# dyollb/segmantic

Measured on AMD Instinct MI355X. Metric: 3D UNet train voxels/s on 128^3 bf16, higher is better.
Workload: dtype bf16

## Files before the change

### segmantic_amd/csrc/conv.hip

```cpp
#include "conv_fwd_impl.h"
#include "conv_ring_impl.h"
#include "conv_ks_impl.h"
#include "convt_ps_impl.h"
#include "conv_bnbwd_impl.h"

namespace segmi {

int conv_s2_bnbwd_bf16(const ConvBnBwdParams& p, hipStream_t st);
int conv_s2_bnbwd_f16(const ConvBnBwdParams& p, hipStream_t st);

int conv_mfma_f32(const ConvParams& p, int ksize, int stride, hipStream_t st);
int conv_mfma_bf16(const ConvParams& p, int ksize, int stride, hipStream_t st);
int conv_mfma_f16(const ConvParams& p, int ksize, int stride, hipStream_t st);
int convt_mfma_f32(const ConvTParams& p, hipStream_t st);
int convt_mfma_bf16(const ConvTParams& p, hipStream_t st);
int convt_mfma_f16(const ConvTParams& p, hipStream_t st);
static inline int conv_mfma_dt(int dtype, const ConvParams& p, int ksize, int stride, hipStream_t st) {
  if (dtype == SEGMI_F32) return conv_mfma_f32(p, ksize, stride, st);
  return dtype == SEGMI_F16 ? conv_mfma_f16(p, ksize, stride, st) : conv_mfma_bf16(p, ksize, stride, st);
}
static inline int convt_mfma_dt(int dtype, const ConvTParams& p, hipStream_t st) {
  if (dtype == SEGMI_F32) return convt_mfma_f32(p, st);
  return dtype == SEGMI_F16 ? convt_mfma_f16(p, st) : convt_mfma_bf16(p, st);
}
int bn_stats_launch(int dtype, const segmi_act* x, float* partials, hipStream_t st, const BiasFin* bias_fin = nullptr);
int bn_stats_rows_for(const segmi_act* x);
int stats_reserve_rows();
static inline int bn_finalize_with(const float* partials, int rows, int c, const segmi_bn_fin* f, hipStream_t st) {
  return segmi_bn_finalize(partials, rows, c, f->count, f->gamma, f->beta, f->running_mean, f->running_var,
                           f->momentum, f->eps, f->mean, f->invstd, f->scale, f->shift, st);
}
bool conv_small_ok(int cin, int cout, int ksize);
int conv_small_fwd(int dtype, const segmi_act* in, const segmi_act* out, const float* w,
                   const float* bias, const float* alpha, const segmi_act* res, float* stats,
                   int stride, hipStream_t st, const segmi_act* out2 = nullptr,
                   const float* w2 = nullptr, const float* bias2 = nullptr,
                   const segmi_bn_fin* fin = nullptr, const segmi_windows* win = nullptr);
int conv_small_fwd_rows(const segmi_act* out);

struct DirectParams {
  const void* in;
  void* out;
  const float* w;
  const float* bias;
  const float* alpha;
  const void* res;
  int N, Di, Hi, Wi, Do, Ho, Wo, Cin, Cout, ldi, ldo, ldr;
  int ks, stride, kind;
};

template <typename T>
__global__ void conv_direct_kernel(DirectParams p) {
  const int64_t total = (int64_t)p.N * p.Do * p.Ho * p.Wo * p.Cout;
  const int pad = (p.ks - 1) / 2, nt = p.ks * p.ks * p.ks;
  const T* in = (const T*)p.in;
  for (int64_t e = blockIdx.x * (int64_t)blockDim.x + threadIdx.x; e < total;
       e += (int64_t)gridDim.x * blockDim.x) {
    const int co = e % p.Cout;
    int64_t v = e / p.Cout;
    const int ox = v % p.Wo; v /= p.Wo;
    const int oy = v % p.Ho; v /= p.Ho;
    const int oz = v % p.Do;
    const int n = v / p.Do;
    float acc = 0.f;
    for (int kd = 0; kd < p.ks; ++kd) {
      const int z = oz * p.stride - pad + kd;
      if ((unsigned)z >= (unsigned)p.Di) continue;
      for (int kh = 0; kh < p.ks; ++kh) {
        const int y = oy * p.stride - pad + kh;
        if ((unsigned)y >= (unsigned)p.Hi) continue;
        for (int kw = 0; kw < p.ks; ++kw) {
          const int x = ox * p.stride - pad + kw;
          if ((unsigned)x >= (unsigned)p.Wi) continue;
          const int tap = (kd * p.ks + kh) * p.ks + kw;
          const T* ip = in + ((((int64_t)n * p.Di + z) * p.Hi + y) * p.Wi + x) * p.ldi;
          if (p.kind == 0) {
            const float* wp = p.w + ((int64_t)co * p.Cin) * nt + tap;
            for (int ci = 0; ci < p.Cin; ++ci) acc = fmaf(Elem<T>::ld(ip + ci), wp[(int64_t)ci * nt], acc);
          } else {
            const float* wp = p.w + (int64_t)co * nt + (nt - 1 - tap);
            for (int ci = 0; ci < p.Cin; ++ci)
              acc = fmaf(Elem<T>::ld(ip + ci), wp[(int64_t)ci * p.Cout * nt], acc);
          }
        }
      }
    }
    if (p.bias) acc += p.bias[co];
    if (p.alpha) acc = acc > 0.f ? acc : (*p.alpha) * acc;
    const int64_t vox = (((int64_t)n * p.Do + oz) * p.Ho + oy) * p.Wo + ox;
    if (p.res) acc += Elem<T>::ld((const T*)p.res + vox * p.ldr + co);
    Elem<T>::st((T*)p.out + vox * p.ldo + co, acc);
  }
}

template <typename T>
__global__ void convt_direct_kernel(DirectParams p) {
  const int64_t total = (int64_t)p.N * p.Do * p.Ho * p.Wo * p.Cout;
  const T* in = (const T*)p.in;
  for (int64_t e = blockIdx.x * (int64_t)blockDim.x + threadIdx.x; e < total;
       e += (int64_t)gridDim.x * blockDim.x) {
    const int co = e % p.Cout;
    int64_t v = e / p.Cout;
    const int ox = v % p.Wo; v /= p.Wo;
    const int oy = v % p.Ho; v /= p.Ho;
    const int oz = v % p.Do;
    const int n = v / p.Do;
    float acc = 0.f;
    for (int kd = 0; kd < 3; ++kd) {
      const int tz = oz + 1 - kd;
      if (tz < 0 || (tz & 1) || (tz >> 1) >= p.Di) continue;
      for (int kh = 0; kh < 3; ++kh) {
        const int ty = oy + 1 - kh;
        if (ty < 0 || (ty & 1) || (ty >> 1) >= p.Hi) continue;
        for (int kw = 0; kw < 3; ++kw) {
          const int tx = ox + 1 - kw;
          if (tx < 0 || (tx & 1) || (tx >> 1) >= p.Wi) continue;
          const int tap = (kd * 3 + kh) * 3 + kw;
          const T* ip = in + ((((int64_t)n * p.Di + (tz >> 1)) * p.Hi + (ty >> 1)) * p.Wi + (tx >> 1)) * p.ldi;
          const float* wp = p.w + (int64_t)co * 27 + tap;
          for (int ci = 0; ci < p.Cin; ++ci)
            acc = fmaf(Elem<T>::ld(ip + ci), wp[(int64_t)ci * p.Cout * 27], acc);
        }
      }
    }
    if (p.bias) acc += p.bias[co];
    if (p.alpha) acc = acc > 0.f ? acc : (*p.alpha) * acc;
    const int64_t vox = (((int64_t)n * p.Do + oz) * p.Ho + oy) * p.Wo + ox;
    if (p.res) acc += Elem<T>::ld((const T*)p.res + vox * p.ldr + co);
    Elem<T>::st((T*)p.out + vox * p.ldo + co, acc);
  }
}

static inline bool mfma_ok(int cin, int cout) { return cin % 16 == 0 && cout % 16 == 0; }

static inline int out_extent(int in, int ks, int stride) {
  const int pad = (ks - 1) / 2;
  return (in + 2 * pad - ks) / stride + 1;
}

}

using namespace segmi;

static inline bool small_fwd_eligible(int dtype, const segmi_act* in, const segmi_act* out, int ksize) {
  const int es = dtype_size(dtype);
  return conv_small_ok(in->c, out->c, ksize) && out->ld % 4 == 0 &&
         ((uintptr_t)out->data % (4 * es)) == 0;
}

extern "C" {

int segmi_conv3d_stats_rows(int dtype, const segmi_act* in, const segmi_act* out, int ksize,
                            int stride) {
  if (!in || !out) return 0;
  if (mfma_ok(in->c, out->c)) {
    if (conv_ring_ok(dtype, in->c, ksize, stride, out))
      return conv_ring_rows(dtype, in->c, out) + stats_reserve_rows();
    if (conv_ks_ok(dtype, in->c, ksize, stride)) return conv_ks_rows(out) + stats_reserve_rows();
    return conv_mfma_rows(out, stride) + stats_reserve_rows();
  }
  if (small_fwd_eligible(dtype, in, out, ksize)) return conv_small_fwd_rows(out) + stats_reserve_rows();
  return bn_stats_rows_for(out) + stats_reserve_rows();
}

int segmi_conv3d_pair_ok(int dtype, const segmi_act* in, const segmi_act* out_a,
                         const segmi_act* out_b) {
  if (!act_ok(in) || !act_ok(out_a) || !act_ok(out_b)) return 0;
  if (!dtype_ok(dtype)) return 0;
  return !mfma_ok(in->c, out_a->c) && small_fwd_eligible(dtype, in, out_a, 3) &&
         small_fwd_eligible(dtype, in, out_b, 3) && out_a->c == out_b->c && out_a->n == out_b->n &&
         out_a->d == out_b->d && out_a->h == out_b->h && out_a->w == out_b->w;
}

int segmi_conv3d_fwd_pair(int dtype, const segmi_act* in, const segmi_act* out_a, const float* w_a,
                          const float* bias_a, const float* prelu_alpha_a, float* stats_partials_a,
                          const segmi_act* out_b, const float* w_b, const float* bias_b, int stride,
                          const segmi_bn_fin* stats_fin_a, const segmi_windows* windows, void* stream) {
  SEGMI_CHECK_ARG(!stats_fin_a || (stats_partials_a && bn_fin_ok(stats_fin_a)),
                  "conv3d_fwd_pair: stats_fin_a needs stats_partials_a and its output pointers");
  if (windows) {
    const int es = dtype_size(dtype);
    bool ok = in && in->c == 1 && in->ld == 1 && windows->count == in->n && windows->count >= 1 && windows->count <= 32 &&
              windows->row_stride >= in->w && windows->row_stride % 4 == 0 && in->w % 4 == 0 &&
              windows->plane_stride >= (int64_t)windows->row_stride * in->h && windows->plane_stride % 4 == 0 &&
              ((uintptr_t)in->data % (4 * es)) == 0;
    for (int i = 0; ok && i < windows->count; ++i) ok = windows->offset[i] >= 0 && windows->offset[i] % 4 == 0;
    SEGMI_CHECK_ARG(ok, "conv3d_fwd_pair: bad window views (single channel, <= 32 windows, 4-element aligned "
                        "offsets and strides)");
  }
  SEGMI_CHECK_ARG(segmi_conv3d_pair_ok(dtype, in, out_a, out_b),
                  "conv3d_fwd_pair: not a small-Cin k3 pair (ask segmi_conv3d_pair_ok first)");
  SEGMI_CHECK_ARG(w_a && w_b && (stride == 1 || stride == 2), "conv3d_fwd_pair: bad arguments");
  SEGMI_CHECK_ARG(in->n == out_a->n && out_a->d == out_extent(in->d, 3, stride) &&
                      out_a->h == out_extent(in->h, 3, stride) && out_a->w == out_extent(in->w, 3, stride),
                  "conv3d_fwd_pair: output extent does not match the input");
  SEGMI_CHECK_ARG(!(stats_partials_a && prelu_alpha_a),
                  "conv3d_fwd_pair: fused statistics are taken before PReLU");
  return conv_small_fwd(dtype, in, out_a, w_a, bias_a, prelu_alpha_a, nullptr, stats_partials_a,
                        stride, (hipStream_t)stream, out_b, w_b, bias_b, stats_fin_a, windows);
}

int segmi_conv3d_split_act_ok(int dtype, const segmi_act* in, const segmi_act* out, int ksize,
                              int stride) {
  if (!act_ok(in) || !act_ok(out) || !dtype_ok(dtype)) return 0;
  return mfma_ok(in->c, out->c) && ksize == 3 && stride == 2 && !conv_ks_ok(dtype, in->c, ksize, stride) &&
         !conv_ring_ok(dtype, in->c, ksize, stride, out);
}

int segmi_conv3d_fwd_split_act(int dtype, const segmi_act* in, const segmi_act* out, const void* packed,
                               const float* bias, const float* prelu_alpha, int act_channels, int ksize,
                               int stride, const float* bias_b, float* stats_partials,
                               const segmi_bn_fin* stats_fin, void* stream) {
  SEGMI_CHECK_ARG(segmi_conv3d_split_act_ok(dtype, in, out, ksize, stride),
                  "conv3d_fwd_split_act: layer not eligible (ask segmi_conv3d_split_act_ok)");
  SEGMI_CHECK_ARG(packed && act_channels > 0 && act_channels % 16 == 0 && act_channels <= out->c,
                  "conv3d_fwd_split_act: act_channels must be a multiple of 16 within the output channels");
  SEGMI_CHECK_ARG(in->n == out->n && out->d == out_extent(in->d, ksize, stride) &&
                      out->h == out_extent(in->h, ksize, stride) && out->w == out_extent(in->w, ksize, stride),
                  "conv3d_fwd_split_act: output extent does not match the input");
  const int es = dtype_size(dtype);
  SEGMI_CHECK_ARG(in->ld % (16 / es) == 0 && out->ld % 4 == 0 && ((uintptr_t)in->data % 16) == 0 &&
                      ((uintptr_t)out->data % (4 * es)) == 0,
                  "conv3d_fwd_split_act: MFMA path needs 16-byte aligned input rows");
  ConvParams p{};
  p.in = in->data; p.out = out->data; p.wfrag = packed; p.bias = bias; p.alpha = prelu_alpha;
  p.N = in->n; p.Di = in->d; p.Hi = in->h; p.Wi = in->w;
  p.Do = out->d; p.Ho = out->h; p.Wo = out->w;
  p.Cin = in->c; p.Cout = out->c; p.ldi = in->ld; p.ldo = out->ld;
  p.nchunks = in->c / pick_ck(dtype, in->c);
  p.ntiles_total = out->c / 16;
  p.act_tiles = act_channels / 16;
  p.bias2 = bias_b;
  if (stats_partials) {
    p.stats = stats_partials;
    p.stats_tiles = act_channels / 16;
    if (stats_fin) { p.fin_on = 1; p.bfin = bn_fin_from(stats_fin, act_channels); }
  } else {
    SEGMI_CHECK_ARG(!stats_fin, "conv3d_fwd_split_act: stats_fin needs stats_partials");
  }
  hipStream_t st = (hipStream_t)stream;
  return conv_mfma_dt(dtype, p, ksize, stride, st);
}

const char* segmi_conv3d_fwd_kernel_name(int dtype, const segmi_act* in, const segmi_act* out,
                                         int ksize, int stride) {
  static thread_local char buf[96];
  if (!act_ok(in) || !act_ok(out)) return "invalid";
  const char* dt = dtype == SEGMI_BF16 ? "bf16" : dtype == SEGMI_F16 ? "f16" : "f32";
  if (mfma_ok(in->c, out->c)) {
    const int ck = pick_ck(dtype, in->c);
    if (conv_ring_ok(dtype, in->c, ksize, stride, out)) {
      if (conv_ring3_shape_ok(in->c, out->c, in->data, out->data, in->d, in->h, in->w, in->ld, out->d, out->h, out->w, out->ld,
                              out->ld, out->ld))
        snprintf(buf, sizeof buf, "conv_ring3_kernel<%s, CK=16> (LDS-DMA ring)", dt);
      else
        snprintf(buf, sizeof buf, "conv_ring2_kernel<%s, CK=%d, NT=%d>", dt, ck,
                 ck == 32 && (out->c / 16) % 2 == 0 ? 2 : 1);
    }
    else if (conv_ks_ok(dtype, in->c, ksize, stride))
      snprintf(buf, sizeof buf, "conv_fwd_ks_kernel<%s, k%d s%d>", dt, ksize, stride);
    else
      snprintf(buf, sizeof buf, "conv_fwd_mfma_kernel<%s, CK=%d, k%d s%d>", dt, ck, ksize, stride);
    return buf;
  }
  if (small_fwd_eligible(dtype, in, out, ksize)) snprintf(buf, sizeof buf, "conv_small_fwd_kernel<%s>", dt);
  else snprintf(buf, sizeof buf, "conv_direct_kernel<%s>", dt);
  return buf;
}

int segmi_conv3d_in_affine_ok(int dtype, const segmi_act* in, const segmi_act* out, int ksize,
                              int stride) {
  if (!act_ok(in) || !act_ok(out) || !dtype_h16(dtype) || !mfma_ok(in->c, out->c)) return 0;
  return ksize == 3 && stride == 1 && conv_ring_ok(dtype, in->c, ksize, stride, out) ? 1 : 0;
}

int segmi_conv3d_bn_bwd_sums_ok(int dtype, const segmi_act* in, const segmi_act* out, int ksize,
                                int stride) {
  if (!act_ok(in) || !act_ok(out) || !dtype_h16(dtype)) return 0;
  return ((in->c == 16 && out->c == 16) || (in->c == 32 && out->c == 32)) && ksize == 3 && stride == 1 &&
                 conv_ring_ok(dtype, in->c, ksize, stride, out) ? 1 : 0;
}

int segmi_bn_act_bwd_apply_conv_ok(int dtype, const segmi_act* dy, const segmi_act* x, const segmi_act* dx,
                                   const segmi_act* out) {
  if (!dtype_h16(dtype) || !act_ok(dy) || !act_ok(x) || !act_ok(dx) || !act_ok(out)) return 0;
  const segmi_act* a3[3] = {dy, x, dx};
  for (const segmi_act* a : a3) {
    if (a->n != dy->n || a->d != dy->d || a->h != dy->h || a->w != dy->w || a->c != 16) return 0;
    if (a->ld % 8 != 0 || ((uintptr_t)a->data % 16) != 0) return 0;
  }
  if (out->n != dy->n || out->d != out_extent(dy->d, 3, 2) || out->h != out_extent(dy->h, 3, 2) ||
      out->w != out_extent(dy->w, 3, 2))
    return 0;
  if (!(out->c == 16 || out->c == 32 || out->c == 64) || out->ld % 4 != 0 || ((uintptr_t)out->data % 8) != 0)
    return 0;
  const int64_t vox = (int64_t)dy->d * dy->h * dy->w;
  if (vox * dy->ld * 2 >= (1ll << 31) || vox * x->ld * 2 >= (1ll << 31) || vox * dx->ld * 2 >= (1ll << 31)) return 0;
  return out->w >= 16 ? 1 : 0;
}

int segmi_bn_act_bwd_apply_conv(int dtype, const segmi_act* dy, const segmi_act* x, const segmi_act* dx,
                                const float* mean, const float* invstd, const float* gamma, const float* beta,
                                const float* prelu_alpha, const float* coef, const segmi_act* out,
                                const void* packed, void* stream) {
  SEGMI_CHECK_ARG(segmi_bn_act_bwd_apply_conv_ok(dtype, dy, x, dx, out) && mean && invstd && coef && packed,
                  "bn_act_bwd_apply_conv: not eligible (ask segmi_bn_act_bwd_apply_conv_ok) or bad arguments");
  SEGMI_CHECK_ARG(dx->data != dy->data && dx->data != x->data,
                  "bn_act_bwd_apply_conv: dx must not alias dy or x (halo voxels are re-read by neighbouring tiles)");
  ConvBnBwdParams p{};
  p.dy = dy->data; p.x = x->data; p.dx = dx->data; p.out = out->data; p.wfrag = packed;
  p.mean = mean; p.invstd = invstd; p.gamma = gamma; p.beta = beta; p.alpha = prelu_alpha; p.coef = coef;
  p.N = dy->n; p.Di = dy->d; p.Hi = dy->h; p.Wi = dy->w; p.Do = out->d; p.Ho = out->h; p.Wo = out->w;
  p.Cout = out->c; p.ldy = dy->ld; p.ldx = x->ld; p.lddx = dx->ld; p.ldo = out->ld;
  p.ntiles_total = out->c / 16;
  return dtype == SEGMI_F16 ? conv_s2_bnbwd_f16(p, (hipStream_t)stream) : conv_s2_bnbwd_bf16(p, (hipStream_t)stream);
}

int segmi_conv3d_fwd(int dtype, const segmi_act* in, const segmi_act* out, const void* packed,
                     const float* w_src, int w_kind, const float* bias,
                     const float* prelu_alpha, const segmi_act* residual,
                     float* stats_partials, int ksize, int stride, const segmi_in_affine* in_tf,
                     const segmi_bn_bwd_sums* bn_bwd, const segmi_bn_fin* stats_fin, void* stream) {
  SEGMI_CHECK_ARG(!stats_fin || (stats_partials && bn_fin_ok(stats_fin)),
                  "conv3d: stats_fin needs stats_partials and its output pointers");
  if (bn_bwd && bn_bwd->fin)
    SEGMI_CHECK_ARG(bn_bwd->fin->count > 0 && bn_bwd->fin->coef, "conv3d: bn_bwd->fin needs count and coef");
  if (bn_bwd)
    SEGMI_CHECK_ARG(bn_bwd->x && act_ok(bn_bwd->x) && bn_bwd->mean && bn_bwd->invstd && bn_bwd->partials &&
                        segmi_conv3d_bn_bwd_sums_ok(dtype, in, out, ksize, stride) && !prelu_alpha &&
                        !stats_partials && bn_bwd->x->n == out->n && bn_bwd->x->d == out->d &&
                        bn_bwd->x->h == out->h && bn_bwd->x->w == out->w && bn_bwd->x->c == out->c &&
                        bn_bwd->x->ld % 4 == 0 && ((uintptr_t)bn_bwd->x->data % 8) == 0,
                    "conv3d: this launch cannot take BatchNorm-backward sums (ask segmi_conv3d_bn_bwd_sums_ok)");
  if (in_tf)
    SEGMI_CHECK_ARG(in_tf->scale && in_tf->shift && segmi_conv3d_in_affine_ok(dtype, in, out, ksize, stride),
                    "conv3d: this layer cannot take an input transform (ask segmi_conv3d_in_affine_ok)");
  SEGMI_CHECK_ARG(dtype_ok(dtype), "conv3d: bad dtype %d", dtype);
  SEGMI_CHECK_ARG(act_ok(in) && act_ok(out), "conv3d: bad activation view");
  SEGMI_CHECK_ARG((ksize == 1 || ksize == 3) && (stride == 1 || stride == 2),
                  "conv3d: unsupported ksize/stride %d/%d", ksize, stride);
  SEGMI_CHECK_ARG(!(ksize == 1 && stride != 1), "conv3d: k1 is stride 1 only");
  SEGMI_CHECK_ARG(in->n == out->n && out->d == out_extent(in->d, ksize, stride) &&
                      out->h == out_extent(in->h, ksize, stride) &&
                      out->w == out_extent(in->w, ksize, stride),
                  "conv3d: output extent [%d,%d,%d,%d] does not match input [%d,%d,%d,%d] k%d s%d",
                  out->n, out->d, out->h, out->w, in->n, in->d, in->h, in->w, ksize, stride);
  if (residual)
    SEGMI_CHECK_ARG(act_ok(residual) && residual->n == out->n && residual->d == out->d &&
                        residual->h == out->h && residual->w == out->w && residual->c == out->c,
                    "conv3d: residual shape mismatch");
  hipStream_t st = (hipStream_t)stream;
  const int es = dtype_size(dtype);
  if (mfma_ok(in->c, out->c)) {
    SEGMI_CHECK_ARG(packed, "conv3d: MFMA path needs a fragment-packed weight (segmi_wpack)");
    SEGMI_CHECK_ARG(in->ld % (16 / es) == 0 && out->ld % 4 == 0 &&
                        ((uintptr_t)in->data % 16) == 0 && ((uintptr_t)out->data % (4 * es)) == 0,
                    "conv3d: MFMA path needs 16-byte aligned input rows");
    if (residual)
      SEGMI_CHECK_ARG(residual->ld % 4 == 0 && ((uintptr_t)residual->data % (4 * es)) == 0,
                      "conv3d: residual rows must be 4-element aligned");
    ConvParams p{};
    p.in = in->data; p.out = out->data; p.wfrag = packed; p.bias = bias; p.alpha = prelu_alpha;
    p.res = residual ? residual->data : nullptr; p.stats = stats_partials;
    p.N = in->n; p.Di = in->d; p.Hi = in->h; p.Wi = in->w;
    p.Do = out->d; p.Ho = out->h; p.Wo = out->w;
    p.Cin = in->c; p.Cout = out->c; p.ldi = in->ld; p.ldo = out->ld;
    p.ldr = residual ? residual->ld : 0;
    p.nchunks = in->c / pick_ck(dtype, in->c);
    p.ntiles_total = out->c / 16;
    if (in_tf) { p.in_scale = in_tf->scale; p.in_shift = in_tf->shift; p.in_alpha = in_tf->prelu_alpha; }
    if (bn_bwd) {
      p.bx = bn_bwd->x->data; p.ldbx = bn_bwd->x->ld; p.bmean = bn_bwd->mean; p.binvstd = bn_bwd->invstd;
      p.bgamma = bn_bwd->gamma; p.bbeta = bn_bwd->beta; p.balpha = bn_bwd->prelu_alpha;
      p.bpart = bn_bwd->partials;
      SEGMI_CHECK_ARG((int64_t)p.Ho * p.Wo * p.ldbx < (1ll << 31), "conv3d: plane too large for 32-bit offsets");
      if (bn_bwd->fin) {
        p.fin_on = 1;
        p.bbfin = BnBwdFin{out->c, bn_bwd->fin->count, bn_bwd->fin->dgamma, bn_bwd->fin->dbeta,
                           bn_bwd->fin->dalpha, bn_bwd->fin->coef};
      }
    }
    if (stats_fin) { p.fin_on = 1; p.bfin = bn_fin_from(stats_fin, out->c); }
    return conv_mfma_dt(dtype, p, ksize, stride, st);
  }
  SEGMI_CHECK_ARG(w_src, "conv3d: direct path (channels not multiples of 16) needs w_src");
  SEGMI_CHECK_ARG(w_kind == 0 || w_kind == 1, "conv3d: bad w_kind %d", w_kind);
  SEGMI_CHECK_ARG(!(stats_partials && small_fwd_eligible(dtype, in, out, ksize) && w_kind != 0),
                  "conv3d: fused statistics on a small-Cin layer need the forward weight kind");
  if (small_fwd_eligible(dtype, in, out, ksize) && w_kind == 0 &&
      (!residual || (residual->ld % 4 == 0 && ((uintptr_t)residual->data % (4 * es)) == 0))) {
    SEGMI_CHECK_ARG(!stats_partials || (!prelu_alpha && !residual),
                    "conv3d: fused statistics are taken before PReLU/residual");
    return conv_small_fwd(dtype, in, out, w_src, bias, prelu_alpha, residual, stats_partials, stride,
                          st, nullptr, nullptr, nullptr, stats_fin);
  }
  DirectParams p{};
  p.in = in->data; p.out = out->data; p.w = w_src; p.bias = bias; p.alpha = prelu_alpha;
  p.res = residual ? residual->data : nullptr;
  p.N = in->n; p.Di = in->d; p.Hi = in->h; p.Wi = in->w; p.Do = out->d; p.Ho = out->h;
  p.Wo = out->w; p.Cin = in->c; p.Cout = out->c; p.ldi = in->ld; p.ldo = out->ld;
  p.ldr = residual ? residual->ld : 0; p.ks = ksize; p.stride = stride; p.kind = w_kind;
  const int64_t total = act_voxels(out) * out->c;
  int blocks = (int)(cdiv64(total, 256) > 8192 ? 8192 : cdiv64(total, 256));
  if (dtype == SEGMI_F32) hipLaunchKernelGGL(conv_direct_kernel<float>, blocks, 256, 0, st, p);
  else if (dtype == SEGMI_F16) hipLaunchKernelGGL(conv_direct_kernel<f16_t>, blocks, 256, 0, st, p);
  else hipLaunchKernelGGL(conv_direct_kernel<bf16_t>, blocks, 256, 0, st, p);
  SEGMI_LAUNCH_CHECK("conv3d_fwd(direct)");
  if (stats_partials) {
    SEGMI_CHECK_ARG(!prelu_alpha && !residual,
                    "conv3d: fused statistics are taken before PReLU/residual");
    const int rc = bn_stats_launch(dtype, out, stats_partials, st);
    if (rc != SEGMI_OK || !stats_fin) return rc;
    return bn_finalize_with(stats_partials, segmi_conv3d_stats_rows(dtype, in, out, ksize, stride), out->c,
                            stats_fin, st);
  }
  return SEGMI_OK;
}

int segmi_convT3d_stats_rows(int dtype, const segmi_act* in, const segmi_act* out) {
  if (!in || !out) return 0;
  if (mfma_ok(in->c, out->c)) return convt_mfma_rows(dtype, in, out->c) + stats_reserve_rows();
  return bn_stats_rows_for(out) + stats_reserve_rows();
}

int segmi_convT3d_fwd(int dtype, const segmi_act* in, const segmi_act* out, const void* packed,
                      const float* w_src, const float* bias, const float* prelu_alpha,
                      const segmi_act* residual, float* stats_partials, const segmi_bn_fin* stats_fin,
                      void* stream) {
  SEGMI_CHECK_ARG(!stats_fin || (stats_partials && bn_fin_ok(stats_fin)),
                  "convT3d: stats_fin needs stats_partials and its output pointers");
  SEGMI_CHECK_ARG(dtype_ok(dtype), "convT3d: bad dtype %d", dtype);
  SEGMI_CHECK_ARG(act_ok(in) && act_ok(out), "convT3d: bad activation view");
  SEGMI_CHECK_ARG(in->n == out->n, "convT3d: batch mismatch");
  const int di[3] = {in->d, in->h, in->w}, dout[3] = {out->d, out->h, out->w};
  for (int k = 0; k < 3; ++k)
    SEGMI_CHECK_ARG(dout[k] == 2 * di[k] || dout[k] == 2 * di[k] - 1,
                    "convT3d: output extent %d must be 2*in or 2*in-1 (in %d)", dout[k], di[k]);
  if (residual)
    SEGMI_CHECK_ARG(act_ok(residual) && residual->n == out->n && residual->d == out->d &&
                        residual->h == out->h && residual->w == out->w && residual->c == out->c,
                    "convT3d: residual shape mismatch");
  hipStream_t st = (hipStream_t)stream;
  const int es = dtype_size(dtype);
  if (mfma_ok(in->c, out->c)) {
    SEGMI_CHECK_ARG(packed, "convT3d: MFMA path needs a kind-2 fragment pack (segmi_wpack)");
    SEGMI_CHECK_ARG(in->ld % (16 / es) == 0 && out->ld % 4 == 0 &&
                        ((uintptr_t)in->data % 16) == 0 && ((uintptr_t)out->data % (4 * es)) == 0,
                    "convT3d: MFMA path needs 16-byte aligned input rows");
    if (residual)
      SEGMI_CHECK_ARG(residual->ld % 4 == 0 && ((uintptr_t)residual->data % (4 * es)) == 0,
                      "convT3d: residual rows must be 4-element aligned");
    ConvTParams p{};
    p.in = in->data; p.out = out->data; p.wfrag = packed; p.bias = bias; p.alpha = prelu_alpha;
    p.res = residual ? residual->data : nullptr; p.stats = stats_partials;
    p.N = in->n; p.Di = in->d; p.Hi = in->h; p.Wi = in->w;
    p.Do = out->d; p.Ho = out->h; p.Wo = out->w;
    p.Cin = in->c; p.Cout = out->c; p.ldi = in->ld; p.ldo = out->ld;
    p.ldr = residual ? residual->ld : 0;
    p.nchunks = in->c / pick_ck(dtype, in->c);
    p.ntiles_total = out->c / 16;
    if (stats_fin) { p.fin_on = 1; p.bfin = bn_fin_from(stats_fin, out->c); }
    return convt_mfma_dt(dtype, p, st);
  }
  SEGMI_CHECK_ARG(w_src, "convT3d: direct path (channels not multiples of 16) needs w_src");
  DirectParams p{};
  p.in = in->data; p.out = out->data; p.w = w_src; p.bias = bias; p.alpha = prelu_alpha;
  p.res = residual ? residual->data : nullptr;
  p.N = in->n; p.Di = in->d; p.Hi = in->h; p.Wi = in->w; p.Do = out->d; p.Ho = out->h;
  p.Wo = out->w; p.Cin = in->c; p.Cout = out->c; p.ldi = in->ld; p.ldo = out->ld;
  p.ldr = residual ? residual->ld : 0; p.ks = 3; p.stride = 2; p.kind = 2;
  const int64_t total = act_voxels(out) * out->c;
  int blocks = (int)(cdiv64(total, 256) > 8192 ? 8192 : cdiv64(total, 256));
  if (dtype == SEGMI_F32) hipLaunchKernelGGL(convt_direct_kernel<float>, blocks, 256, 0, st, p);
  else if (dtype == SEGMI_F16) hipLaunchKernelGGL(convt_direct_kernel<f16_t>, blocks, 256, 0, st, p);
  else hipLaunchKernelGGL(convt_direct_kernel<bf16_t>, blocks, 256, 0, st, p);
  SEGMI_LAUNCH_CHECK("convT3d_fwd(direct)");
  if (stats_partials) {
    SEGMI_CHECK_ARG(!prelu_alpha && !residual,
                    "convT3d: fused statistics are taken before PReLU/residual");
    const int rc = bn_stats_launch(dtype, out, stats_partials, st);
    if (rc != SEGMI_OK || !stats_fin) return rc;
    return bn_finalize_with(stats_partials, segmi_convT3d_stats_rows(dtype, in, out), out->c, stats_fin, st);
  }
  return SEGMI_OK;
}

}
```

### segmantic_amd/csrc/conv_ks_impl.h

```cpp
#pragma once
#include "conv_fwd_impl.h"

namespace segmi {

template <typename T, int CK, int KS, int S, int NT, int TD, int TH, int TW>
__global__ __launch_bounds__(256) void conv_fwd_ks_kernel(ConvParams p) {
  using G = ConvGeom<T, CK, KS, S, TD, TH, TW>;
  static_assert(G::SPT == 4, "k-split kernel: one k-step per tap");
  static_assert(G::NVT == 8, "k-split kernel: 8 voxel tiles per workgroup");
  constexpr int NSW = (G::NSTEP + 3) / 4;
  extern __shared__ __attribute__((aligned(16))) char smem[];
  const int tid = threadIdx.x, lane = tid & 63;
  const int wave = __builtin_amdgcn_readfirstlane(tid >> 6);
  const int g = lane >> 4, r = lane & 15;

  int t = blockIdx.x;
  const int txi = t % p.tx; t /= p.tx;
  const int tyi = t % p.ty; t /= p.ty;
  const int tzi = t % p.tz;
  const int n = t / p.tz;
  const int oz0 = tzi * TD, oy0 = tyi * TH, ox0 = txi * TW;
  const int iz0 = oz0 * S - G::PAD, iy0 = oy0 * S - G::PAD, ix0 = ox0 * S - G::PAD;
  const int nt0 = blockIdx.y * NT;

  f32x4 acc[8][NT];
#pragma unroll
  for (int i = 0; i < 8; ++i)
#pragma unroll
    for (int j = 0; j < NT; ++j) acc[i][j] = f32x4{0.f, 0.f, 0.f, 0.f};

  int vaddr[8];
#pragma unroll
  for (int i = 0; i < 8; ++i) {
    const int idx = i * 16 + r;
    const int x = idx % TW, y = (idx / TW) % TH, z = idx / (TW * TH);
    vaddr[i] = ((z * S * G::HH + y * S) * G::HW + x * S) * G::ROWB + g * 16;
  }
  int tapoff[NSW];
#pragma unroll
  for (int si = 0; si < NSW; ++si) {
    int tap = wave + 4 * si;
    if (tap > G::NTAPS - 1) tap = G::NTAPS - 1;
    tapoff[si] = (((tap / (KS * KS)) * G::HH + (tap / KS) % KS) * G::HW + tap % KS) * G::ROWB;
  }

  constexpr int NCH = G::HD * G::HH * G::HW * G::CPR;
  constexpr int NLD = (NCH + 255) / 256;
  const char* inb = (const char*)p.in;
  frag_t stg[NLD];
  auto fetch = [&](int c) {
#pragma unroll
    for (int k = 0; k < NLD; ++k) {
      const int i = tid + 256 * k;
      const int v = i / G::CPR, ch = i % G::CPR;
      const int hx = v % G::HW, hy = (v / G::HW) % G::HH, hz = v / (G::HW * G::HH);
      const int z = iz0 + hz, y = iy0 + hy, x = ix0 + hx;
      stg[k] = frag_t{0u, 0u, 0u, 0u};
      if (i < NCH && (unsigned)z < (unsigned)p.Di && (unsigned)y < (unsigned)p.Hi &&
          (unsigned)x < (unsigned)p.Wi) {
        const int64_t e = ((((int64_t)n * p.Di + z) * p.Hi + y) * p.Wi + x) * p.ldi + c * CK;
        stg[k] = *reinterpret_cast<const frag_t*>(inb + e * (int64_t)sizeof(T) + ch * 16);
      }
    }
  };
  const char* wb0 = (const char*)p.wfrag + (int64_t)nt0 * 1024 + lane * 16;
  frag_t wcur[NSW][NT], wnxt[NSW][NT];
  auto fetch_w = [&](int c, frag_t (&dst)[NSW][NT]) {
#pragma unroll
    for (int si = 0; si < NSW; ++si) {
      int s = wave + 4 * si;
      if (s > G::NSTEP - 1) s = G::NSTEP - 1;
#pragma unroll
      for (int j = 0; j < NT; ++j)
        dst[si][j] = *reinterpret_cast<const frag_t*>(
            wb0 + (((int64_t)c * G::NSTEP + s) * p.ntiles_total + j) * 1024);
    }
  };
  fetch(0);
  fetch_w(0, wcur);
  for (int c = 0; c < p.nchunks; ++c) {
    if (c > 0) __syncthreads();
#pragma unroll
    for (int k = 0; k < NLD; ++k) {
      const int i = tid + 256 * k;
      if (i < NCH) *reinterpret_cast<frag_t*>(smem + (i / G::CPR) * G::ROWB + (i % G::CPR) * 16) = stg[k];
    }
    __syncthreads();
    if (c + 1 < p.nchunks) {
      fetch(c + 1);
      fetch_w(c + 1, wnxt);
    }
#pragma unroll
    for (int si = 0; si < NSW; ++si) {
      const int s = wave + 4 * si;
      if (s < G::NSTEP) {
#pragma unroll
        for (int i = 0; i < 8; ++i) {
          const frag_t a = *reinterpret_cast<const frag_t*>(smem + vaddr[i] + tapoff[si]);
#pragma unroll
          for (int j = 0; j < NT; ++j) acc[i][j] = mma16<T>(wcur[si][j], a, acc[i][j]);
        }
      }
    }
#pragma unroll
    for (int si = 0; si < NSW; ++si)
#pragma unroll
      for (int j = 0; j < NT; ++j) wcur[si][j] = wnxt[si][j];
  }

  __syncthreads();
  f32x4* red = reinterpret_cast<f32x4*>(smem);
#pragma unroll
  for (int i = 0; i < 8; ++i)
#pragma unroll
    for (int j = 0; j < NT; ++j) red[((wave * 8 + i) * NT + j) * 64 + lane] = acc[i][j];
  __syncthreads();
  f32x4 fin[2][NT];
#pragma unroll
  for (int ii = 0; ii < 2; ++ii)
#pragma unroll
    for (int j = 0; j < NT; ++j) {
      const int i = wave * 2 + ii;
      f32x4 v = red[((0 * 8 + i) * NT + j) * 64 + lane];
      v += red[((1 * 8 + i) * NT + j) * 64 + lane];
      v += red[((2 * 8 + i) * NT + j) * 64 + lane];
      v += red[((3 * 8 + i) * NT + j) * 64 + lane];
      fin[ii][j] = v;
    }

  f32x4 bias4[NT];
#pragma unroll
  for (int j = 0; j < NT; ++j) {
    bias4[j] = f32x4{0.f, 0.f, 0.f, 0.f};
    if (p.bias) bias4[j] = *reinterpret_cast<const f32x4*>(p.bias + (nt0 + j) * 16 + 4 * g);
  }
  const bool has_alpha = p.alpha != nullptr;
  const float alpha = has_alpha ? *p.alpha : 0.f;
  f32x4 ssum[NT], ssq[NT];
#pragma unroll
  for (int j = 0; j < NT; ++j) {
    ssum[j] = f32x4{0.f, 0.f, 0.f, 0.f};
    ssq[j] = f32x4{0.f, 0.f, 0.f, 0.f};
  }
  T* outp = (T*)p.out;
  const T* resp = (const T*)p.res;
  f32x4 resv[2][NT];
  if (resp) {
#pragma unroll
    for (int ii = 0; ii < 2; ++ii) {
      const int idx = (wave * 2 + ii) * 16 + r;
      const int oz = oz0 + idx / (TW * TH), oy = oy0 + (idx / TW) % TH, ox = ox0 + idx % TW;
      const bool valid = oz < p.Do && oy < p.Ho && ox < p.Wo;
      const int64_t vox = (((int64_t)n * p.Do + oz) * p.Ho + oy) * p.Wo + ox;
#pragma unroll
      for (int j = 0; j < NT; ++j)
        resv[ii][j] = valid ? load4<T>(resp + vox * p.ldr + (nt0 + j) * 16 + 4 * g)
                            : f32x4{0.f, 0.f, 0.f, 0.f};
    }
#pragma unroll
    for (int ii = 0; ii < 2; ++ii)
#pragma unroll
      for (int j = 0; j < NT; ++j) touch_v(resv[ii][j]);
  }
#pragma unroll
  for (int j = 0; j < NT; ++j) touch_v(bias4[j]);
#pragma unroll
  for (int k = 0; k < NLD; ++k) touch_v(stg[k]);
#pragma unroll
  for (int ii = 0; ii < 2; ++ii) {
    const int idx = (wave * 2 + ii) * 16 + r;
    const int oz = oz0 + idx / (TW * TH), oy = oy0 + (idx / TW) % TH, ox = ox0 + idx % TW;
    const bool valid = oz < p.Do && oy < p.Ho && ox < p.Wo;
    const int64_t vox = (((int64_t)n * p.Do + oz) * p.Ho + oy) * p.Wo + ox;
#pragma unroll
    for (int j = 0; j < NT; ++j) {
      f32x4 v = fin[ii][j] + bias4[j];
      if (valid) {
        if (p.stats) {
          ssum[j] += v;
          ssq[j] += v * v;
        }
        if (has_alpha) {
#pragma unroll
          for (int e = 0; e < 4; ++e) v[e] = v[e] > 0.f ? v[e] : alpha * v[e];
        }
        const int co = (nt0 + j) * 16 + 4 * g;
        if (resp) v += resv[ii][j];
        store4<T>(outp + vox * p.ldo + co, v);
      }
    }
  }
  if (p.stats) {
    __syncthreads();
    float* rs = reinterpret_cast<float*>(smem);
#pragma unroll
    for (int j = 0; j < NT; ++j)
#pragma unroll
      for (int e = 0; e < 4; ++e) {
        const float a = row16_sum(ssum[j][e]);
        const float b = row16_sum(ssq[j][e]);
        if (r == 0) {
          rs[(wave * 2 + 0) * NT * 16 + j * 16 + 4 * g + e] = a;
          rs[(wave * 2 + 1) * NT * 16 + j * 16 + 4 * g + e] = b;
        }
      }
    __syncthreads();
    if (tid < 2 * NT * 16) {
      const int which = tid / (NT * 16), ch = tid % (NT * 16);
      float sacc = 0.f;
#pragma unroll
      for (int w = 0; w < 4; ++w) sacc += rs[(w * 2 + which) * NT * 16 + ch];
      fin_store(&p.stats[((int64_t)blockIdx.x * 2 + which) * p.Cout + nt0 * 16 + ch], sacc);
    }
    fin_tail_run<BnFin, 256, offsetof(ConvParams, ft), offsetof(ConvParams, bfin)>(p.stats, smem);
  }
}

template <typename T, int CK, int KS, int S, int NT, int TD, int TH, int TW>
static int launch_conv_ks_cfg(ConvParams p, hipStream_t st) {
  using G = ConvGeom<T, CK, KS, S, TD, TH, TW>;
  p.tz = cdiv(p.Do, TD);
  p.ty = cdiv(p.Ho, TH);
  p.tx = cdiv(p.Wo, TW);
  const int64_t nb = (int64_t)p.N * p.tz * p.ty * p.tx;
  SEGMI_CHECK_ARG(nb < (1ll << 31), "conv3d: too many tiles");
  dim3 grid((unsigned)nb, (unsigned)(p.Cout / (16 * NT)));
  constexpr int red = 4 * 8 * NT * 64 * 16;
  constexpr int lds0 = G::LDS_BYTES > red ? G::LDS_BYTES : red;
  p.fin_on = p.fin_on && p.stats;
  const int lds = (int)fin_tail_arm(p, grid, 256, 2 * p.Cout, lds0);
  auto kern = conv_fwd_ks_kernel<T, CK, KS, S, NT, TD, TH, TW>;
  static bool attr_done = false;
  if (!attr_done && lds > 64 * 1024) {
    (void)hipFuncSetAttribute(reinterpret_cast<const void*>(kern),
                              hipFuncAttributeMaxDynamicSharedMemorySize, lds);
    attr_done = true;
  }
  hipLaunchKernelGGL(kern, grid, 256, lds, st, p);
  SEGMI_LAUNCH_CHECK("conv3d_fwd(mfma, k-split)");
  return SEGMI_OK;
}

static inline int conv_ks_rows(const segmi_act* out) {
  const bool wide = out->w > 8;
  const int td = wide ? 2 : 4, th = 4, tw = wide ? 16 : 8;
  return out->n * cdiv(out->d, td) * cdiv(out->h, th) * cdiv(out->w, tw);
}
static inline bool conv_ks_ok(int dtype, int cin, int ksize, int stride) {
  static const bool off = getenv("SEGMI_CONV_KS") && atoi(getenv("SEGMI_CONV_KS")) == 0;
  static const bool one = !(getenv("SEGMI_CONV_KS_1CH") && atoi(getenv("SEGMI_CONV_KS_1CH")) == 0);
  if (off || ksize != 3 || stride != 1) return false;
  const int ck = pick_ck(dtype, cin);
  const int spt = ck / (dtype == SEGMI_F32 ? 4 : 8);
  return spt == 4 && cin / ck >= (one ? 1 : 2);
}

template <typename T, int CK>
static int launch_conv_ks_t(const ConvParams& p, hipStream_t st) {
  const segmi_act o{nullptr, p.N, p.Do, p.Ho, p.Wo, p.Cout, p.Cout};
  const int nt = p.Cout / 16;
  const bool two = nt % 2 == 0 && (int64_t)conv_ks_rows(&o) * (nt / 2) >= 512;
  const bool wide = p.Wo > 8;
  if (two) return wide ? launch_conv_ks_cfg<T, CK, 3, 1, 2, 2, 4, 16>(p, st)
                       : launch_conv_ks_cfg<T, CK, 3, 1, 2, 4, 4, 8>(p, st);
  return wide ? launch_conv_ks_cfg<T, CK, 3, 1, 1, 2, 4, 16>(p, st)
              : launch_conv_ks_cfg<T, CK, 3, 1, 1, 4, 4, 8>(p, st);
}

}
```

### segmantic_amd/csrc/conv_mfma_h16.h

```cpp
#pragma once
#include "conv_fwd_impl.h"
#include "conv_ring2_impl.h"
#include "conv_ring3_impl.h"
#include "conv_ks_impl.h"
#include "convt_ps_impl.h"
#include "conv_bnbwd_impl.h"
namespace segmi {
template <typename T>
static int conv_mfma_h16(const ConvParams& p, int ksize, int stride, hipStream_t st) {
  constexpr int dt = DtypeOf<T>::value;
  if (conv_ring_zsplit(dt, p.Cin, ksize, stride, p.N, p.Do, p.Ho, p.Wo) > 0)
    return conv_ring3_ok(p) ? launch_conv_ring3<T>(p, st) : launch_conv_ring2<T>(p, st);
  if (conv_ks_ok(dt, p.Cin, ksize, stride)) return launch_conv_ks_t<T, 32>(p, st);
  return launch_conv_mfma_t<T>(p, ksize, stride, st);
}
template <typename T>
static int conv_s2_bnbwd_h16(const ConvBnBwdParams& p, hipStream_t st) {
  switch (p.Cout / 16) {
    case 1: return launch_conv_s2_bnbwd<T, 1>(p, st);
    case 2: return launch_conv_s2_bnbwd<T, 2>(p, st);
    case 4: return launch_conv_s2_bnbwd<T, 4>(p, st);
  }
  SEGMI_UNSUPPORTED("bn_act_bwd_apply_conv: %d output channels", p.Cout);
}
template <typename T>
static int convt_mfma_h16(const ConvTParams& p, hipStream_t st) {
  if (convt_ps_ok(DtypeOf<T>::value, p.Cin, p.Cout, p.Wi)) return launch_convt_ps_t<T>(p, st);
  return launch_convt_mfma_t<T>(p, st);
}
}
```

Measured before the change: 3.567 billion.

## Add persistent pipelined k-split conv kernel prefetching next tile into registers

Adds a persistent variant of the k-split 3x3x3 conv forward kernel. Grid size is set from occupancy times CU count, and each workgroup walks a contiguous range of output tiles. While MFMAs run on the current tile, the next tile's input halo is prefetched into registers, hiding global load latency and cutting launch and tail overhead. In exchange it raises register pressure (launch_bounds 256,2) and adds extra syncs per tile. It is used by default for single-chunk h16 layers.

Result: no change. 3.557 billion, median of 3 (-0.3%).

```diff
diff --git a/segmantic_amd/csrc/conv.hip b/segmantic_amd/csrc/conv.hip
--- a/segmantic_amd/csrc/conv.hip
+++ b/segmantic_amd/csrc/conv.hip
@@ -1,6 +1,6 @@
 #include "conv_fwd_impl.h"
 #include "conv_ring_impl.h"
-#include "conv_ks_impl.h"
+#include "conv_ks_pipe_impl.h"
 #include "convt_ps_impl.h"
 #include "conv_bnbwd_impl.h"
 
@@ -258,7 +258,9 @@
                  ck == 32 && (out->c / 16) % 2 == 0 ? 2 : 1);
     }
     else if (conv_ks_ok(dtype, in->c, ksize, stride))
-      snprintf(buf, sizeof buf, "conv_fwd_ks_kernel<%s, k%d s%d>", dt, ksize, stride);
+      snprintf(buf, sizeof buf, "%s<%s, k%d s%d>",
+               dtype_h16(dtype) && in->c == ck && conv_ks_pipe_on() ? "conv_fwd_ks_pipe_kernel" : "conv_fwd_ks_kernel",
+               dt, ksize, stride);
     else
       snprintf(buf, sizeof buf, "conv_fwd_mfma_kernel<%s, CK=%d, k%d s%d>", dt, ck, ksize, stride);
     return buf;
diff --git a/segmantic_amd/csrc/conv_ks_impl.h b/segmantic_amd/csrc/conv_ks_impl.h
--- a/segmantic_amd/csrc/conv_ks_impl.h
+++ b/segmantic_amd/csrc/conv_ks_impl.h
@@ -255,11 +255,15 @@
   return spt == 4 && cin / ck >= (one ? 1 : 2);
 }
 
+static inline bool conv_ks_two(const ConvParams& p) {
+  const segmi_act o{nullptr, p.N, p.Do, p.Ho, p.Wo, p.Cout, p.Cout};
+  const int nt = p.Cout / 16;
+  return nt % 2 == 0 && (int64_t)conv_ks_rows(&o) * (nt / 2) >= 512;
+}
+
 template <typename T, int CK>
 static int launch_conv_ks_t(const ConvParams& p, hipStream_t st) {
-  const segmi_act o{nullptr, p.N, p.Do, p.Ho, p.Wo, p.Cout, p.Cout};
-  const int nt = p.Cout / 16;
-  const bool two = nt % 2 == 0 && (int64_t)conv_ks_rows(&o) * (nt / 2) >= 512;
+  const bool two = conv_ks_two(p);
   const bool wide = p.Wo > 8;
   if (two) return wide ? launch_conv_ks_cfg<T, CK, 3, 1, 2, 2, 4, 16>(p, st)
                        : launch_conv_ks_cfg<T, CK, 3, 1, 2, 4, 4, 8>(p, st);
diff --git a/segmantic_amd/csrc/conv_ks_pipe_impl.h b/segmantic_amd/csrc/conv_ks_pipe_impl.h
--- /dev/null
+++ b/segmantic_amd/csrc/conv_ks_pipe_impl.h
@@ -0,0 +1,285 @@
+#pragma once
+#include <atomic>
+#include "conv_ks_impl.h"
+
+namespace segmi {
+
+template <typename T, int CK, int KS, int S, int NT, int TD, int TH, int TW>
+__global__ __launch_bounds__(256, 2) void conv_fwd_ks_pipe_kernel(ConvParams p) {
+  using G = ConvGeom<T, CK, KS, S, TD, TH, TW>;
+  static_assert(G::SPT == 4, "k-split kernel: one k-step per tap");
+  static_assert(G::NVT == 8, "k-split kernel: 8 voxel tiles per workgroup");
+  constexpr int NSW = (G::NSTEP + 3) / 4;
+  extern __shared__ __attribute__((aligned(16))) char smem[];
+  const int tid = threadIdx.x, lane = tid & 63;
+  const int wave = __builtin_amdgcn_readfirstlane(tid >> 6);
+  const int g = lane >> 4, r = lane & 15;
+
+  const int nb = p.N * p.tz * p.ty * p.tx;
+  const int t_begin = (int)((int64_t)blockIdx.x * nb / gridDim.x);
+  const int t_end = (int)((int64_t)(blockIdx.x + 1) * nb / gridDim.x);
+  const int nt0 = blockIdx.y * NT;
+
+  int vaddr[8];
+#pragma unroll
+  for (int i = 0; i < 8; ++i) {
+    const int idx = i * 16 + r;
+    const int x = idx % TW, y = (idx / TW) % TH, z = idx / (TW * TH);
+    vaddr[i] = ((z * S * G::HH + y * S) * G::HW + x * S) * G::ROWB + g * 16;
+  }
+  int tapoff[NSW];
+#pragma unroll
+  for (int si = 0; si < NSW; ++si) {
+    int tap = wave + 4 * si;
+    if (tap > G::NTAPS - 1) tap = G::NTAPS - 1;
+    tapoff[si] = (((tap / (KS * KS)) * G::HH + (tap / KS) % KS) * G::HW + tap % KS) * G::ROWB;
+  }
+
+  constexpr int NCH = G::HD * G::HH * G::HW * G::CPR;
+  constexpr int NLD = (NCH + 255) / 256;
+  const char* inb = (const char*)p.in;
+  frag_t stg[NLD];
+  auto fetch = [&](int t) {
+    const int txi = t % p.tx, tyi = (t / p.tx) % p.ty, tzi = (t / (p.tx * p.ty)) % p.tz;
+    const int n = t / (p.tx * p.ty * p.tz);
+    const int iz0 = tzi * TD * S - G::PAD, iy0 = tyi * TH * S - G::PAD, ix0 = txi * TW * S - G::PAD;
+#pragma unroll
+    for (int k = 0; k < NLD; ++k) {
+      const int i = tid + 256 * k;
+      const int v = i / G::CPR, ch = i % G::CPR;
+      const int hx = v % G::HW, hy = (v / G::HW) % G::HH, hz = v / (G::HW * G::HH);
+      const int z = iz0 + hz, y = iy0 + hy, x = ix0 + hx;
+      stg[k] = frag_t{0u, 0u, 0u, 0u};
+      if (i < NCH && (unsigned)z < (unsigned)p.Di && (unsigned)y < (unsigned)p.Hi &&
+          (unsigned)x < (unsigned)p.Wi) {
+        const int64_t e = ((((int64_t)n * p.Di + z) * p.Hi + y) * p.Wi + x) * p.ldi;
+        stg[k] = *reinterpret_cast<const frag_t*>(inb + e * (int64_t)sizeof(T) + ch * 16);
+      }
+    }
+  };
+  const char* wb0 = (const char*)p.wfrag + (int64_t)nt0 * 1024 + lane * 16;
+  frag_t wcur[NSW][NT];
+#pragma unroll
+  for (int si = 0; si < NSW; ++si) {
+    int s = wave + 4 * si;
+    if (s > G::NSTEP - 1) s = G::NSTEP - 1;
+#pragma unroll
+    for (int j = 0; j < NT; ++j)
+      wcur[si][j] = *reinterpret_cast<const frag_t*>(wb0 + ((int64_t)s * p.ntiles_total + j) * 1024);
+  }
+
+  const bool has_alpha = p.alpha != nullptr;
+  const float alpha = has_alpha ? *p.alpha : 0.f;
+  T* outp = (T*)p.out;
+  const T* resp = (const T*)p.res;
+
+  if (t_begin < t_end) fetch(t_begin);
+  for (int t = t_begin; t < t_end; ++t) {
+    const int txi = t % p.tx, tyi = (t / p.tx) % p.ty, tzi = (t / (p.tx * p.ty)) % p.tz;
+    const int n = t / (p.tx * p.ty * p.tz);
+    const int oz0 = tzi * TD, oy0 = tyi * TH, ox0 = txi * TW;
+
+    f32x4 acc[8][NT];
+#pragma unroll
+    for (int i = 0; i < 8; ++i)
+#pragma unroll
+      for (int j = 0; j < NT; ++j) acc[i][j] = f32x4{0.f, 0.f, 0.f, 0.f};
+
+    __syncthreads();
+#pragma unroll
+    for (int k = 0; k < NLD; ++k) {
+      const int i = tid + 256 * k;
+      if (i < NCH) *reinterpret_cast<frag_t*>(smem + (i / G::CPR) * G::ROWB + (i % G::CPR) * 16) = stg[k];
+    }
+    __syncthreads();
+    if (t + 1 < t_end) fetch(t + 1);
+#pragma unroll
+    for (int si = 0; si < NSW; ++si) {
+      const int s = wave + 4 * si;
+      if (s < G::NSTEP) {
+#pragma unroll
+        for (int i = 0; i < 8; ++i) {
+          const frag_t a = *reinterpret_cast<const frag_t*>(smem + vaddr[i] + tapoff[si]);
+#pragma unroll
+          for (int j = 0; j < NT; ++j) acc[i][j] = mma16<T>(wcur[si][j], a, acc[i][j]);
+        }
+      }
+    }
+
+    __syncthreads();
+    f32x4* red = reinterpret_cast<f32x4*>(smem);
+#pragma unroll
+    for (int i = 0; i < 8; ++i)
+#pragma unroll
+      for (int j = 0; j < NT; ++j) red[((wave * 8 + i) * NT + j) * 64 + lane] = acc[i][j];
+    __syncthreads();
+    f32x4 fin[2][NT];
+#pragma unroll
+    for (int ii = 0; ii < 2; ++ii)
+#pragma unroll
+      for (int j = 0; j < NT; ++j) {
+        const int i = wave * 2 + ii;
+        f32x4 v = red[((0 * 8 + i) * NT + j) * 64 + lane];
+        v += red[((1 * 8 + i) * NT + j) * 64 + lane];
+        v += red[((2 * 8 + i) * NT + j) * 64 + lane];
+        v += red[((3 * 8 + i) * NT + j) * 64 + lane];
+        fin[ii][j] = v;
+      }
+
+    f32x4 bias4[NT];
+#pragma unroll
+    for (int j = 0; j < NT; ++j) {
+      bias4[j] = f32x4{0.f, 0.f, 0.f, 0.f};
+      if (p.bias) bias4[j] = *reinterpret_cast<const f32x4*>(p.bias + (nt0 + j) * 16 + 4 * g);
+    }
+    f32x4 ssum[NT], ssq[NT];
+#pragma unroll
+    for (int j = 0; j < NT; ++j) {
+      ssum[j] = f32x4{0.f, 0.f, 0.f, 0.f};
+      ssq[j] = f32x4{0.f, 0.f, 0.f, 0.f};
+    }
+    f32x4 resv[2][NT];
+    if (resp) {
+#pragma unroll
+      for (int ii = 0; ii < 2; ++ii) {
+        const int idx = (wave * 2 + ii) * 16 + r;
+        const int oz = oz0 + idx / (TW * TH), oy = oy0 + (idx / TW) % TH, ox = ox0 + idx % TW;
+        const bool valid = oz < p.Do && oy < p.Ho && ox < p.Wo;
+        const int64_t vox = (((int64_t)n * p.Do + oz) * p.Ho + oy) * p.Wo + ox;
+#pragma unroll
+        for (int j = 0; j < NT; ++j)
+          resv[ii][j] = valid ? load4<T>(resp + vox * p.ldr + (nt0 + j) * 16 + 4 * g)
+                              : f32x4{0.f, 0.f, 0.f, 0.f};
+      }
+#pragma unroll
+      for (int ii = 0; ii < 2; ++ii)
+#pragma unroll
+        for (int j = 0; j < NT; ++j) touch_v(resv[ii][j]);
+    }
+#pragma unroll
+    for (int j = 0; j < NT; ++j) touch_v(bias4[j]);
+#pragma unroll
+    for (int k = 0; k < NLD; ++k) touch_v(stg[k]);
+#pragma unroll
+    for (int ii = 0; ii < 2; ++ii) {
+      const int idx = (wave * 2 + ii) * 16 + r;
+      const int oz = oz0 + idx / (TW * TH), oy = oy0 + (idx / TW) % TH, ox = ox0 + idx % TW;
+      const bool valid = oz < p.Do && oy < p.Ho && ox < p.Wo;
+      const int64_t vox = (((int64_t)n * p.Do + oz) * p.Ho + oy) * p.Wo + ox;
+#pragma unroll
+      for (int j = 0; j < NT; ++j) {
+        f32x4 v = fin[ii][j] + bias4[j];
+        if (valid) {
+          if (p.stats) {
+            ssum[j] += v;
+            ssq[j] += v * v;
+          }
+          if (has_alpha) {
+#pragma unroll
+            for (int e = 0; e < 4; ++e) v[e] = v[e] > 0.f ? v[e] : alpha * v[e];
+          }
+          const int co = (nt0 + j) * 16 + 4 * g;
+          if (resp) v += resv[ii][j];
+          store4<T>(outp + vox * p.ldo + co, v);
+        }
+      }
+    }
+    if (p.stats) {
+      __syncthreads();
+      float* rs = reinterpret_cast<float*>(smem);
+#pragma unroll
+      for (int j = 0; j < NT; ++j)
+#pragma unroll
+        for (int e = 0; e < 4; ++e) {
+          const float a = row16_sum(ssum[j][e]);
+          const float b = row16_sum(ssq[j][e]);
+          if (r == 0) {
+            rs[(wave * 2 + 0) * NT * 16 + j * 16 + 4 * g + e] = a;
+            rs[(wave * 2 + 1) * NT * 16 + j * 16 + 4 * g + e] = b;
+          }
+        }
+      __syncthreads();
+      if (tid < 2 * NT * 16) {
+        const int which = tid / (NT * 16), ch = tid % (NT * 16);
+        float sacc = 0.f;
+#pragma unroll
+        for (int w = 0; w < 4; ++w) sacc += rs[(w * 2 + which) * NT * 16 + ch];
+        fin_store(&p.stats[((int64_t)t * 2 + which) * p.Cout + nt0 * 16 + ch], sacc);
+      }
+    }
+  }
+  if (p.stats)
+    fin_tail_run<BnFin, 256, offsetof(ConvParams, ft), offsetof(ConvParams, bfin)>(p.stats, smem);
+}
+
+template <class K>
+static int conv_ks_pipe_capacity(K kern, int lds) {
+  static std::atomic<int> cache[16];
+  int dev = 0;
+  if (hipGetDevice(&dev) != hipSuccess) return 0;
+  if (dev >= 0 && dev < 16) {
+    const int c = cache[dev].load(std::memory_order_relaxed);
+    if (c > 0) return c;
+  }
+  int per_cu = 0, cus = 0;
+  if (hipOccupancyMaxActiveBlocksPerMultiprocessor(&per_cu, reinterpret_cast<const void*>(kern), 256, lds) !=
+      hipSuccess)
+    per_cu = 0;
+  if (hipDeviceGetAttribute(&cus, hipDeviceAttributeMultiprocessorCount, dev) != hipSuccess) cus = 0;
+  (void)hipGetLastError();
+  const int cap = per_cu * cus;
+  if (dev >= 0 && dev < 16 && cap > 0) cache[dev].store(cap, std::memory_order_relaxed);
+  return cap;
+}
+
+template <typename T, int CK, int KS, int S, int NT, int TD, int TH, int TW>
+static int launch_conv_ks_pipe_cfg(ConvParams p, hipStream_t st) {
+  using G = ConvGeom<T, CK, KS, S, TD, TH, TW>;
+  p.tz = cdiv(p.Do, TD);
+  p.ty = cdiv(p.Ho, TH);
+  p.tx = cdiv(p.Wo, TW);
+  const int64_t nb = (int64_t)p.N * p.tz * p.ty * p.tx;
+  SEGMI_CHECK_ARG(nb < (1ll << 31), "conv3d: too many tiles");
+  const int gy = p.Cout / (16 * NT);
+  constexpr int red = 4 * 8 * NT * 64 * 16;
+  constexpr int lds0 = G::LDS_BYTES > red ? G::LDS_BYTES : red;
+  p.fin_on = p.fin_on && p.stats;
+  size_t lds = lds0;
+  auto kern = conv_fwd_ks_pipe_kernel<T, CK, KS, S, NT, TD, TH, TW>;
+  if (p.fin_on) {
+    const size_t need = fin_tail_lds(2 * p.Cout, 256);
+    if (need > lds) lds = need;
+  }
+  static bool attr_done = false;
+  if (!attr_done && lds > 64 * 1024) {
+    (void)hipFuncSetAttribute(reinterpret_cast<const void*>(kern),
+                              hipFuncAttributeMaxDynamicSharedMemorySize, (int)lds);
+    attr_done = true;
+  }
+  int64_t gx = conv_ks_pipe_capacity(kern, (int)lds) / gy;
+  if (gx < 1) gx = 1;
+  if (gx > nb) gx = nb;
+  const dim3 grid((unsigned)gx, (unsigned)gy);
+  if (p.fin_on) p.ft = fin_tail_make((int)nb, 2 * p.Cout, grid.x * grid.y);
+  else p.ft.on = 0;
+  hipLaunchKernelGGL(kern, grid, 256, lds, st, p);
+  SEGMI_LAUNCH_CHECK("conv3d_fwd(mfma, k-split, pipelined)");
+  return SEGMI_OK;
+}
+
+static inline bool conv_ks_pipe_on() {
+  static const bool off = getenv("SEGMI_CONV_KS_PIPE") && atoi(getenv("SEGMI_CONV_KS_PIPE")) == 0;
+  return !off;
+}
+
+template <typename T, int CK>
+static int launch_conv_ks_pipe_t(const ConvParams& p, hipStream_t st) {
+  SEGMI_CHECK_ARG(p.nchunks == 1, "conv3d: the pipelined k-split kernel takes single-chunk layers only");
+  const bool two = conv_ks_two(p), wide = p.Wo > 8;
+  if (two) return wide ? launch_conv_ks_pipe_cfg<T, CK, 3, 1, 2, 2, 4, 16>(p, st)
+                       : launch_conv_ks_pipe_cfg<T, CK, 3, 1, 2, 4, 4, 8>(p, st);
+  return wide ? launch_conv_ks_pipe_cfg<T, CK, 3, 1, 1, 2, 4, 16>(p, st)
+              : launch_conv_ks_pipe_cfg<T, CK, 3, 1, 1, 4, 4, 8>(p, st);
+}
+
+}
diff --git a/segmantic_amd/csrc/conv_mfma_h16.h b/segmantic_amd/csrc/conv_mfma_h16.h
--- a/segmantic_amd/csrc/conv_mfma_h16.h
+++ b/segmantic_amd/csrc/conv_mfma_h16.h
@@ -2,7 +2,7 @@
 #include "conv_fwd_impl.h"
 #include "conv_ring2_impl.h"
 #include "conv_ring3_impl.h"
-#include "conv_ks_impl.h"
+#include "conv_ks_pipe_impl.h"
 #include "convt_ps_impl.h"
 #include "conv_bnbwd_impl.h"
 namespace segmi {
@@ -11,7 +11,8 @@
   constexpr int dt = DtypeOf<T>::value;
   if (conv_ring_zsplit(dt, p.Cin, ksize, stride, p.N, p.Do, p.Ho, p.Wo) > 0)
     return conv_ring3_ok(p) ? launch_conv_ring3<T>(p, st) : launch_conv_ring2<T>(p, st);
-  if (conv_ks_ok(dt, p.Cin, ksize, stride)) return launch_conv_ks_t<T, 32>(p, st);
+  if (conv_ks_ok(dt, p.Cin, ksize, stride))
+    return conv_ks_pipe_on() && p.nchunks == 1 ? launch_conv_ks_pipe_t<T, 32>(p, st) : launch_conv_ks_t<T, 32>(p, st);
   return launch_conv_mfma_t<T>(p, ksize, stride, st);
 }
 template <typename T>
```
